# gabraham/flashpca

Measured on AMD Instinct MI355X. Metric: genotype cells/sec (N x P x iters) for k=20 PCA, higher is better.
Workload: dtype i8 (integer genotypes x 7 byte slices of the f64 operand; exact i32 accumulation, f64 recombination; agrees with the f64 kernels to ~3e-15, see fp64_mode); 1 GPU; cfg3: synthetic 500000 samples x 100000 SNPs total, SNP-sharded across GPUs, k=20 (BASELINE configs[2]/[3]); samples=500000, snps_total=100000, snps_per_gpu=100000, k=20, blockvec=16, solver_default_blockvec=16, parallelism=snp-shard x1 + all-reduce(N x b) [single]

## Files before the change

### flashpca_amd/_lib.py

```python
import ctypes as C
import os
import subprocess

HERE = os.path.dirname(os.path.abspath(__file__))
LIB_PATH = os.environ.get("FPCA_LIB") or os.path.join(HERE, "_build", "libfpca.so")
if LIB_PATH == "testhooks":
    LIB_PATH = os.path.join(HERE, "_build", "testhooks", "libfpca.so")
CLI_PATH = os.path.join(HERE, "_build", "flashpca")
HOOKS_LIB_PATH = os.path.join(HERE, "_build", "testhooks", "libfpca.so")
HOOKS_CLI_PATH = os.path.join(HERE, "_build", "testhooks", "flashpca")
CSRC = os.path.join(HERE, "csrc")

STANDARDISE = {"binom": 2, "binom2": 3}
STANDARDISE_DENSE = {"none": 0, "sd": 1, "binom": 2, "binom2": 3, "center": 4}
DIVISOR = {"none": 0, "n1": 1, "p": 2}
UNIQUE_ID_BYTES = 128
SCCA_STATUS = {0: "ok", 1: "maxiter reached", 2: "lambda1 too large", 3: "lambda2 too large"}

ALLREDUCE_FN = C.CFUNCTYPE(C.c_int, C.c_void_p, C.c_void_p, C.c_uint64, C.c_void_p)
COLLECTIVE_FN = C.CFUNCTYPE(C.c_int, C.c_void_p, C.c_void_p, C.c_void_p, C.c_uint64, C.c_void_p)


class PcaOpts(C.Structure):
    _fields_ = [
# ... 119 lines not shown
    "fpca_set_total_snps": (_I, [_P, _U64]),
    "fpca_set_rank": (_I, [_P, _I, _I]),
    "fpca_collective_stats": (_I, [_P, C.POINTER(_U64), C.POINTER(_U64)]),
    "fpca_pca_init_opts": (None, [C.POINTER(PcaOpts), C.c_size_t, C.c_size_t]),
    "fpca_pca_row_ranges": (_I, [_P, C.POINTER(PcaOpts), C.POINTER(_U64), _I]),
    "fpca_pca": (_I, [_P, C.POINTER(PcaOpts), _P, _P, _P, _P, _P, _P, C.POINTER(PcaInfo)]),
    "fpca_check": (_I, [_P, _P, C.c_int64, _P, _I, _I, _P, C.POINTER(_D), C.POINTER(_D)]),
    "fpca_ucca": (_I, [_P, _P, C.c_int64, _I, _I, _P, C.c_int64]),
    "fpca_scca_prepare": (_I, [_P, _P, C.c_int64, _I, _I, _I]),
    "fpca_scca_fit": (_I, [_P, _D, _D, _I, _I, _D, _P, C.c_int64, _P, C.c_int64, _P, C.c_int64, _P, _P, C.c_int64, _P, C.c_int64,
                           C.POINTER(_I), _P, _P, _P, C.POINTER(_I)]),
    "fpca_scca_cv": (_I, [_P, _P, C.c_int64, _I, _P, _I, _P, _I, _P, _I, _I, _I, _I, _I, _D, _P, C.c_int64, C.c_int64, _D, _I, _P, _P, _P, _P, _P, _P,
                          C.POINTER(_D), C.POINTER(_D), C.POINTER(_D), _P, _P]),
    "fpca_bench_apply": (_I, [_P, _I, _I, _I, C.POINTER(BenchResult)]),
    "fpca_profile_begin": (_I, [_P, _I]),
    "fpca_profile_sample_every": (_I, [_P, _I]),
    "fpca_profile_end": (_I, [_P, _I, C.POINTER(BenchResult), C.POINTER(_I)]),
    "fpca_bench_stats": (_I, [_P, _I, C.POINTER(_D), C.POINTER(_D)]),
    "fpca_debug_mfma_probe": (_I, [_P, _P, _P]),
    "fpca_debug_mfma_i8_probe": (_I, [_P, _P, _P]),
    "fpca_debug_mfma_peak": (_I, [_I, _I, _I, C.POINTER(_D)]),
    "fpca_debug_k4": (_I, [_P, _I, _I, _P, _P, _P, _P, _I, _P, _P]),
    "fpca_debug_k4_bench": (_I, [_P, _I, _I, _I, C.POINTER(_D), C.POINTER(_D)]),
    "fpca_debug_k4_fused": (_I, [_P, _I, _I, _P, _P, _P, _P, _P]),
    "fpca_debug_k4_fused_bench": (_I, [_P, _I, _I, _I, C.POINTER(_D)]),
    "fpca_debug_k4_inplace": (_I, [_P, _I, _I, _P, _P, _P, _I, _P, _P]),
    "fpca_debug_fp_plan": (_I, [_P, _I, C.POINTER(_I)]),
    "fpca_debug_poison_partials": (_I, [_P]),
    "fpca_debug_missing_lists": (_I, [_P, _I, _I, _P, _P, _U64, C.POINTER(_U64)]),
    "fpca_debug_gather": (_I, [_I, _I, _P, _P, _U64, _P, _U64, _P, _P, _P, _U64, _U64, _I, _D, _P, C.POINTER(_I)]),
    "fpca_debug_i8_nsc_pad": (_I, [_I, _I, C.POINTER(_I)]),
    "fpca_debug_i8_slices": (_I, [_I, _I, _I, _U64, _U64, _U64, _P, _P, _P, _P, _I, C.POINTER(SlicesOut), C.POINTER(SlicesOut), C.POINTER(_I)]),
    "fpca_debug_i8_instances": (_I, [_P, _I, C.POINTER(_I)]),
    "fpca_debug_f_sf":(_I, [_D, _U64, _I, C.POINTER(_D), C.POINTER(_D)]),
    "fpca_debug_f_sf_dev": (_I, [_P, _U64, _U64, _I, _P, _P]),
    "fpca_debug_scca_lds": (_I, [_I, C.POINTER(_I), C.POINTER(_I), C.POINTER(_I)]),
    "fpca_debug_fold_stats": (_I, [_P, _P, _I, _P, _I, _P]),
    "fpca_debug_snp_qc_rule": (_I, [_P, _P, _U64, _U64, _D, _D, _P, C.POINTER(_U64)]),
    "fpca_debug_snp_subset_bench": (_I, [_P, _P, _I, C.POINTER(_D), C.POINTER(_D)]),
    "fpca_debug_ld_prune_rule": (_I, [_P, _U64, C.c_uint32, C.c_uint32, _P, _P, _P, _P, C.POINTER(_U64)]),
    "fpca_bench_ld": (_I, [_P, C.c_uint32, _I, _P, C.POINTER(_D)]),
    "fpca_debug_king_rule": (_I, [_P, _P, _U64, _U64, _P, C.POINTER(_U64)]),
    "fpca_bench_king": (_I, [_P, _I, _P, C.POINTER(_D)]),
    "fpca_bench_king_rel": (_I, [_P, _I, _P, C.POINTER(_D)]),
    "fpca_debug_sample_qc_rule": (_I, [_P, _U64, _U64, _D, _P, C.POINTER(_U64)]),
    "fpca_debug_snp_qc_counts_rule": (_I, [_P, _P, _U64, _U64, _D, _D, _D, _P, C.POINTER(_U64)]),
    "fpca_bench_qc": (_I, [_P, _I, _P, C.POINTER(_D)]),
    "fpca_debug_scratch_live": (_I, [C.POINTER(_U64)]),
    "fpca_debug_scratch_fail_at": (_I, [_U64]),
}

ABI_VERSION = 4

_lib = None
_loaded = {}


def _load(path):
    if path not in _loaded:
        if not os.path.exists(path):
            raise RuntimeError(
                "%s not found -- build it with `make -C flashpca_amd/csrc` (or __graft_entry__.build()); this package has "
                "no CPU fallback" % path
            )
        L = C.CDLL(path)
        try:
# ... 52 lines not shown
```

### flashpca_amd/api.py

```python
import ctypes as C

import numpy as np

from . import _lib
from ._lib import DIVISOR, STANDARDISE, BenchResult, FpcaError, PcaInfo, PcaOpts, check, lib


ACCUM = {"auto": 0, 0: 0, "fp64": 64, "fp32": 32, 64: 64, 32: 32, "i8": 807}
ACCUM.update({"i8x%d" % s: 800 + s for s in range(2, 9)})
ACCUM.update({800 + s: 800 + s for s in range(2, 9)})


def _p(a):
    return a.ctypes.data_as(C.c_void_p) if a is not None else None


def count_fam_rows(path):
    with open(path, "rb") as f:
        return f.read().count(b"\n")


def _snp_mask(snps, P):
    a = np.asarray(snps)
    if a.dtype == np.bool_:
# ... 580 lines not shown
        a = dict(colmax=np.empty(64), maxbits_own=np.empty((8, 64), dtype=np.uint64), maxbits=np.empty((8, 64), dtype=np.uint64),
                 Q=np.empty((nsc, rows_pad), dtype=np.int8), colw=np.empty(nsc))
        if colsum[o]:
            a["colsum"] = np.empty((8, 640), dtype=np.int64)
        if copy[o] is not None:
            a["copy%d" % copy[o]] = np.empty((rows_pad, b), dtype=np.float32 if copy[o] == 32 else np.float64)
        if route == 1:
            a["Qrm"] = np.empty((rows_pad, S * b), dtype=np.int8)
            for w in dequant:
                a["dq%d" % w] = np.empty((rows_pad, b), dtype=np.float32 if w == 32 else np.float64)
        st = _lib.SlicesOut()
        for name, arr in a.items():
            setattr(st, name, arr.ctypes.data)
        structs.append(st)
        res.append(a)
    got = C.c_int(0)
    check(lib().fpca_debug_i8_slices(int(route), int(b), int(S), rows, rows_pad, int(rows_valid), _p(V), _p(rs[0]) if rs else None,
                                     _p(rs[1]) if len(rs) > 1 else None, _p(peers), 0 if peers is None else peers.shape[0], C.byref(structs[0]),
                                     C.byref(structs[1]) if nops > 1 else None, C.byref(got)))
    for a in res:
        a["nsc_pad"] = got.value
        if "colsum" in a:
            a["colsum_shards"] = a["colsum"]
            a["colsum"] = a["colsum_shards"].sum(axis=0)
    return res


def debug_i8_instances():
    n = C.c_int(0)
    check(lib().fpca_debug_i8_instances(None, 0, C.byref(n)))
    keys = np.zeros((n.value, 6), dtype=np.int32)
    check(lib().fpca_debug_i8_instances(_p(keys), n.value, C.byref(n)))
    return [(bool(k[0]), int(k[1]), int(k[2]), bool(k[3]), int(k[4]), bool(k[5])) for k in keys[:n.value]]


def flashpca(X, ndim=10, stand="binom2", divisor="p", maxiter=500, tol=1e-6, do_loadings=False, return_scale=True,
             device=0, verbose=False, accum="auto", keep=None, snps=None, maf=0.0, geno=1.0, ld=None, unrelated=None,
             mind=1.0, hwe=0.0, unrelated_min_shared=0, **solver_kw):
    if divisor not in DIVISOR:
        raise ValueError("divisor must be one of %s" % sorted(DIVISOR))
    qc = not (maf <= 0 and geno >= 1)
    by_mind, by_hwe = not mind >= 1, not hwe <= 0
    if (snps is not None or qc) and not isinstance(X, str):
        raise ValueError("snps / maf / geno select SNPs of a PLINK fileset; they do not apply to a numeric matrix")
    if (by_mind or by_hwe) and not isinstance(X, str):
        raise ValueError("mind / hwe filter the samples / SNPs of a PLINK fileset; they do not apply to a numeric matrix")
    if qc and keep is not None:
        raise ValueError("maf / geno cannot be combined with keep: PLINK takes these frequencies over the kept samples, the counts here "
                         "are those of all samples")
    if by_hwe and keep is not None:
        raise ValueError("hwe cannot be combined with keep: flashpca() takes the genotype counts over the samples mind= leaves; for a "
                         "hand-picked subset take the masks from qc_filter(..., keep=) and pass them as snps= and keep=")
    if ld is not None:
        ld = _ld_args(ld)
        if not isinstance(X, str):
            raise ValueError("ld prunes the SNPs of a PLINK fileset; it does not apply to a numeric matrix")
        if keep is not None:
            raise ValueError("ld cannot be combined with keep: PLINK takes r2 over the kept samples, r2 here is over all samples")
    if unrelated is not None:
        unrelated = float(unrelated)
        if not isinstance(X, str):
            raise ValueError("unrelated selects samples by the kinship of a PLINK fileset's genotypes; it does not apply to a numeric matrix")
    if isinstance(X, str):
        if stand not in STANDARDISE:
            raise ValueError("stand must be one of %s" % sorted(STANDARDISE))
        N = count_fam_rows(X + ".fam")
# ... 590 lines not shown
```

### flashpca_amd/csrc/kernels.hpp

```cpp
#pragma once
#include <hip/hip_runtime.h>

#include <cstddef>
#include <cstdint>

namespace fpca {
namespace kern {

void repitch(const uint8_t *src, uint64_t np, uint64_t nrec, uint8_t *dst, size_t pitch, hipStream_t stream);
void fix_last_byte(uint8_t *packed, size_t pitch, uint64_t np, int valid_in_last, uint64_t P_g, hipStream_t stream);
void gather_records(const uint8_t *src, size_t pitch, const uint32_t *idx, uint64_t nrec, uint8_t *dst, hipStream_t stream);
void ld_totals(const uint8_t *packed, size_t pitch, uint64_t nrec, uint32_t *tot, hipStream_t stream);
void ld_band(const uint8_t *packed, size_t pitch, const uint32_t *tot, uint32_t npad, uint64_t i0, uint64_t ni, uint64_t jend, uint32_t span,
             double *r2, uint32_t *bits, uint32_t words, double thr, bool force_general, hipStream_t stream);

void bed_stats(const uint8_t *packed, size_t pitch, uint64_t N, uint64_t P_g, int stand_method, double *lut,
               double *mean, double *sd, double *sumsq, uint32_t *nmiss , hipStream_t stream);
void lut_from_meansd(const double *mean, const double *sd, uint64_t P_g, double *lut, hipStream_t stream);

void xt_b(const uint8_t *packed, size_t pitch, const double *lut, const double *B, double *Tpart, uint64_t N_pad,
          uint64_t P_pad, int b, int nsplit, bool fp32, hipStream_t stream);
void x_t(const uint8_t *packed, size_t pitch, const double *lut, const double *T, double *Ypart, uint64_t N_pad,
         uint64_t P_pad, int b, int nsplit, bool fp32, hipStream_t stream);
void reduce_sum(const double *part, double *out, uint64_t count, int nsplit, hipStream_t stream);
// ... 41 lines not shown
                    uint32_t conc_fp = 0, uint64_t med_q32 = 0, uint32_t sig2_fp = 0);

void mfma_layout_probe(const double *A, const double *B, double *D, hipStream_t stream);

double mfma_peak_tflops(int waves_per_simd, int iters, int pattern, hipStream_t stream);

constexpr int I8_SHARDS = 8, I8_CS_STRIDE = 640;
struct SliceOp {
   const double *rowscale;
   unsigned long long *maxbits;
   int8_t *Q;
   double *colw;
   long long *colsum;
   double *copy64;
   float *copy32;
};
void i8_colmax(const double *V, uint64_t rows, int b, int nops, const SliceOp *ops, hipStream_t stream);
void i8_slice(const double *V, uint64_t rows_pad, uint64_t rows, int b, int S, int nops, const SliceOp *ops, hipStream_t stream);
void i8_maxbits_fold(const unsigned long long *bits, double *out64, hipStream_t stream);
void i8_maxbits_set(const double *all, int G, unsigned long long *bits, hipStream_t stream);
void i8_slice_rows(const double *V, uint64_t rows, int b, int S, const SliceOp &op, int8_t *Qrm, hipStream_t stream);
void i8_unpack_slices(const int8_t *Qrm, uint64_t rows_pad, int b, int S, const SliceOp &op, hipStream_t stream, uint64_t rows_valid = 0,
                      float *copy32 = nullptr, double *copy64 = nullptr);
void i8_dequant_rows(const int8_t *Qrm, uint64_t rows, int b, int S, const SliceOp &op, float *copy32, double *copy64, hipStream_t stream);
__host__ __device__ inline size_t packed_piece_offset(uint64_t r, uint64_t q, size_t pitch, bool tiled)
{
   if (!tiled) return (size_t)(r * pitch + q * 16);
   const uint64_t c = q >> 2, kh = (q >> 1) & 1, h = q & 1;
   return (size_t)((r >> 5) * 32 * pitch + c * 2048 + (h * 64 + kh * 32 + (r & 31)) * 16);
}
int gemm_i8_nsc_pad(int S, int b);
size_t gemm_i8_workspace_doubles(uint64_t rows_pad, uint64_t k_pad, int S, int b, bool two);
int gemm_i8_instances(int (*out)[6], int cap);
void gemm_i8(const uint8_t *packed, size_t pitch, const int8_t *Qg, const int8_t *Qm, const double *wg, const double *wm,
             const long long *colsum_m, const double *mean, const double *sd, double *out, double *ws, uint64_t rows_pad, uint64_t k_pad,
             uint64_t rows_valid, int mode ,
             const double *eplane , int b, int S,
             const SliceOp *next_ops, hipStream_t stream, hipEvent_t *gemm_events = nullptr, hipEvent_t before_combine = nullptr,
             bool e_only = false ,
             bool tiled = false );
void i8_rowscales(const double *mean, const double *sd, uint64_t P_g, uint64_t P_pad, double *inv_sd, double *mu_inv_sd,
                  hipStream_t stream);
void transpose_packed(const uint8_t *in, size_t pitch_in, uint64_t N_pad, uint64_t P_pad, uint8_t *out, size_t pitch_out,
                      hipStream_t stream, bool tiled = false );
void tile_packed(const uint8_t *in, size_t pitch, uint64_t rows, uint8_t *out, hipStream_t stream);
double mfma_i8_peak_tops(int waves_per_simd, int iters, uint32_t fill, hipStream_t stream);
void mfma_i8_probe(const int8_t *A, const int8_t *Bt, int *D, hipStream_t stream);

void gather_packed_rows(const uint8_t *src, size_t pitch, const uint32_t *idx, uint32_t nidx, uint32_t rows_out, uint8_t *dst, hipStream_t stream);
void patch_missing_rows(uint8_t *packed, size_t pitch, const uint32_t *idx, uint32_t nidx, hipStream_t stream);
void scatter_packed_rows(const uint8_t *src, size_t pitch, const uint32_t *idx, uint32_t nidx, uint8_t *packed, hipStream_t stream);
void gather_scaled_rows(const double *V, const double *scale, const uint32_t *idx, uint32_t nidx, uint64_t rows_out, int b, double *dst, hipStream_t stream);
void scatter_rows(const double *src, const uint32_t *idx, uint32_t nidx, int b, double *dst, hipStream_t stream);
void count_missing(const uint8_t *packed, size_t pitch, uint64_t ncols, uint64_t nrec, uint32_t *cnt, hipStream_t stream, bool tiled = false);
void fill_missing(const uint8_t *packed, size_t pitch, uint64_t ncols, uint64_t nrec, const uint32_t *ptr, uint32_t *idx, hipStream_t stream,
                  bool tiled = false);
void sparse_rows_sum(const uint32_t *ptr, const uint32_t *idx, const double *V, const double *rowscale, int b, uint64_t nrec,
                     uint64_t rows_out, double *out, hipStream_t stream, const double *init = nullptr ,
                     bool short_lists = false ,
                     double avg_len = 0 );
void sparse_rows_sum_f32(const uint32_t *ptr, const uint32_t *idx, const float *V, const double *colw, int b, uint64_t nrec, uint64_t rows_out,
                         double *out, hipStream_t stream, const double *init = nullptr, bool short_lists = false, double avg_len = 0);
int sparse_rows_sum_variant(int b, bool rowscale, bool short_lists, double avg_len);

}
}
```

### flashpca_amd/csrc/kernels_i8.hip

```cpp
#include <hip/hip_runtime.h>

#include <algorithm>
#include <cmath>
#include <cstdio>
#include <cstdlib>
#include <cstring>
#include <type_traits>
#include <utility>

#include "common.hpp"
#include "dev_scratch.hpp"
#include "kernels.hpp"
#include "launch_check.hpp"

namespace fpca {
namespace kern {

typedef int v4i __attribute__((ext_vector_type(4)));
typedef int v16i __attribute__((ext_vector_type(16)));
typedef double d2 __attribute__((ext_vector_type(2)));
typedef uint32_t u4 __attribute__((ext_vector_type(4)));
typedef uint32_t u2 __attribute__((ext_vector_type(2)));


// ... 1129 lines not shown
static int i8_bw(int b)
{
   return b == 48 ? 96 : std::max(b, 32);
}

static size_t i8_plan_doubles(const I8Plan &p, uint64_t rows_pad, int zb, int bw)
{
   return ((size_t)rows_pad + (size_t)(p.sB - 1) * p.rowsB) * zb * 2 * (size_t)bw;
}

size_t gemm_i8_workspace_doubles(uint64_t rows_pad, uint64_t k_pad, int S, int b, bool two)
{
   size_t need = 0;
   for (int mode : {(int)I8_FULL, (int)I8_SKIP_EMPTY, (int)I8_NO_MISSING}) {
      if (two && mode == I8_NO_MISSING) continue;
      const I8Shape sh = i8_shape(S, b, two, mode, rows_pad);
      const I8Plan p = i8_plan(rows_pad, k_pad, sh, i8_bw(b));
      need = std::max(need, i8_plan_doubles(p, rows_pad, sh.zb, i8_bw(b)));
   }
   return need;
}

template <class C>
static void launch_i8(const I8Plan &pl, hipStream_t stream, const uint8_t *packed, size_t pitch, const int8_t *Qg, const int8_t *Qm,
                      uint64_t k_pad, const double *wg, const double *wm, int bw, double *ws, uint64_t rows_pad, int chunks_total, int zb, uint32_t tab1)
{
   static bool attr_set = false;
   if (!attr_set) {
      (void)hipFuncSetAttribute(reinterpret_cast<const void *>(&k_gemm_i8<C>), hipFuncAttributeMaxDynamicSharedMemorySize, C::LDS_BYTES);
      attr_set = true;
   }
   hipLaunchKernelGGL(HIP_KERNEL_NAME(k_gemm_i8<C>), dim3(pl.grid), dim3(C::THREADS), C::LDS_BYTES, stream, packed, pitch, Qg, Qm, k_pad, wg, wm, bw,
                      ws, rows_pad, chunks_total, zb, pl.nA, pl.sB, pl.cpsB, pl.rowB0, pl.rowsB, tab1);
}

void gemm_i8(const uint8_t *packed, size_t pitch, const int8_t *Qg, const int8_t *Qm, const double *wg, const double *wm,
             const long long *colsum_m, const double *mean, const double *sd, double *out, double *ws, uint64_t rows_pad, uint64_t k_pad,
             uint64_t rows_valid, int mode, const double *eplane , int b,
             int S, const SliceOp *next_ops ,
             hipStream_t stream, hipEvent_t *gemm_events ,
             hipEvent_t before_combine ,
             bool e_only ,
             bool tiled )
{
   const bool two = (Qg != Qm);
   if (tiled && !two && mode != I8_NO_MISSING) throw Error(-1, "gemm_i8: the one-operand kernels of both matrices read the row-major layout only");
   if (tiled && (pitch % 64 || k_pad > 4 * pitch)) throw Error(-1, "gemm_i8: a band-tiled copy has whole 64-byte chunks per row");
   if (e_only && (mode != I8_NO_MISSING || two)) throw Error(-1, "gemm_i8: e_only goes with the one-matrix kernel");
   const I8Shape sh = i8_shape(S, b, two, mode, rows_pad);
   const int bw = i8_bw(b);
   const I8Plan pl = i8_plan(rows_pad, k_pad, sh, bw);
   const int chunks_total = (int)(k_pad / sh.kc);
   const bool nt_p = i8_nt_p(I8Key{two, mode, sh.nt, sh.half, sh.rows, tiled}, e_only);
   if (i8_verbose())
      std::fprintf(stderr, "[fpca] int8 GEMM launch: %s, mode %d, nt %d%s, %s%s; phase B from row %llu; rows %d, loads %s\n", two ? "two operands" : "one operand", mode,
                   sh.nt, sh.half ? " (half tile)" : "", tiled ? "band-tiled" : "row-major", e_only ? ", E alone" : "", (unsigned long long)pl.rowB0,
                   sh.rows, nt_p ? "p" : "plain");
   static const bool poison = FPCA_TEST_ENV("FPCA_DEBUG_I8_POISON") != nullptr;
   if (poison) {
      const size_t used = i8_plan_doubles(pl, rows_pad, sh.zb, bw);
      if (hipMemsetAsync(ws, 0xFF, used * sizeof(double), stream) != hipSuccess) throw Error(-3, "gemm_i8: poisoning the workspace failed");
   }
   if (gemm_events) (void)hipEventRecord(gemm_events[0], stream);
   if (two && mode == I8_NO_MISSING) throw Error(-1, "gemm_i8: without missing genotypes both matrices share one operand (pass Qm == Qg)");
   const bool launched = i8_find(I8Instances{}, I8Key{two, mode, sh.nt, sh.half, sh.rows, tiled, nt_p}, [&](auto c) {
      using C = decltype(c);
// ... 307 lines not shown
```

### flashpca_amd/csrc/missing_kernels.hip

```cpp
#include <hip/hip_runtime.h>

#include <algorithm>
#include <cstdlib>

#include "common.hpp"
#include "kernels.hpp"
#include "launch_check.hpp"

namespace fpca {
namespace kern {

typedef uint32_t u4 __attribute__((ext_vector_type(4)));


__global__ __launch_bounds__(256) void k_count_missing(const uint8_t *__restrict__ packed, size_t pitch, uint64_t ncols,
                                                        uint32_t *__restrict__ cnt, bool tiled)
{
   const uint64_t rec = blockIdx.x;
   auto byte_at = [&](uint64_t j) { return packed + packed_piece_offset(rec, j >> 4, pitch, tiled) + (j & 15); };
   const uint64_t nbytes = (ncols + 3) / 4, nw = nbytes / 4;
   uint32_t n = 0;
   for (uint64_t i = threadIdx.x; i < nw; i += 256) {
      const uint32_t w = *reinterpret_cast<const uint32_t *>(byte_at(4 * i));
      n += __popc(w & ~(w >> 1) & 0x55555555u);
   }
   for (uint64_t i = nw * 4 + threadIdx.x; i < nbytes; i += 256) {
      const uint32_t w = *byte_at(i);
      n += __popc(w & ~(w >> 1) & 0x55u);
   }
   if (threadIdx.x == 0 && (ncols & 3)) {
      const uint32_t w = *byte_at(nbytes - 1) >> (2 * (ncols & 3));
      n -= __popc(w & ~(w >> 1) & 0x55u);
   }
   __shared__ uint32_t red[256];
   red[threadIdx.x] = n;
   __syncthreads();
// ... 219 lines not shown
      uint32_t longest = p1 - p0;
#pragma unroll
      for (int o = 32; o >= B; o >>= 1) longest = max(longest, (uint32_t)__shfl_xor((int)longest, o));
      for (uint32_t base = 0; base < longest; base += B) {
         const uint32_t t = p0 + base + c;
         const int cnt = (int)min((uint32_t)B, p1 - p0 > base ? p1 - p0 - base : 0u);
         const uint32_t mine = t < p1 ? idx[t] : 0u;
#pragma unroll
         for (int e = 0; e < B; e += 4) {
            const uint32_t s0 = (uint32_t)__shfl((int)mine, g * B + e), s1 = (uint32_t)__shfl((int)mine, g * B + e + 1),
                           s2 = (uint32_t)__shfl((int)mine, g * B + e + 2), s3 = (uint32_t)__shfl((int)mine, g * B + e + 3);
            if (e < cnt) a0 += (double)V[(uint64_t)s0 * B + c];
            if (e + 1 < cnt) a1 += (double)V[(uint64_t)s1 * B + c];
            if (e + 2 < cnt) a2 += (double)V[(uint64_t)s2 * B + c];
            if (e + 3 < cnt) a3 += (double)V[(uint64_t)s3 * B + c];
         }
      }
      if (r < rows_out) {
         double a = (a0 + a1) + (a2 + a3);
         if (colw) a *= colw[c] * 32.0;
         out[r * B + c] = init ? init[r * B + c] + a : a;
      }
   }
}

int sparse_rows_sum_variant(int b, bool rowscale, bool short_lists, double avg_len)
{
   static const int forced = FPCA_TEST_ENV("FPCA_GATHER") ? atoi(FPCA_TEST_ENV("FPCA_GATHER")) : 0;
   const int variant = forced ? forced : (avg_len > 0 && avg_len <= 24.0 && b <= 32 && !rowscale) ? 3 : ((rowscale || short_lists) ? 2 : 1);
   if (variant == 3 && b <= 32 && !rowscale) return 3;
   return variant == 1 ? 1 : 2;
}

template <class VT>
static void sparse_rows_sum_t(const uint32_t *ptr, const uint32_t *idx, const VT *V, const double *rowscale, int b, uint64_t nrec,
                              uint64_t rows_out, double *out, hipStream_t stream, const double *init, bool short_lists, const double *colw, double avg_len)
{
   if (!rows_out) return;
   const unsigned blocks = (unsigned)std::min<uint64_t>(65536, (rows_out + 3) / 4);
   const int variant = sparse_rows_sum_variant(b, rowscale != nullptr, short_lists, avg_len);
#define FPCA_GATHER_CASE(B_)                                                                                                    \
   case B_:                                                                                                                     \
      if (variant == 3 && B_ <= 32) {                                                                                           \
         const unsigned blocks3 = (unsigned)std::min<uint64_t>(65536, (rows_out + 4 * (64 / B_) - 1) / (4 * (64 / B_)));        \
         hipLaunchKernelGGL((k_sparse_rows_sum_short<(B_ <= 32 ? B_ : 32), VT>), dim3(blocks3), dim3(256), 0, stream, ptr, idx, V, nrec, rows_out, out, init, colw); \
      } else if (variant == 1)                                                                                                  \
         hipLaunchKernelGGL((k_sparse_rows_sum<B_, VT>), dim3(blocks), dim3(256), 0, stream, ptr, idx, V, rowscale, nrec, rows_out, out, init, colw); \
      else                                                                                                                      \
         hipLaunchKernelGGL((k_sparse_rows_sum_batched<B_, VT>), dim3(blocks), dim3(256), 0, stream, ptr, idx, V, rowscale, nrec, rows_out, out, init, colw); \
      break;
   switch (b) {
      FPCA_GATHER_CASE(16)
      FPCA_GATHER_CASE(32)
      FPCA_GATHER_CASE(64)
   default: throw Error(-1, "sparse_rows_sum: block width must be 16, 32 or 64");
   }
#undef FPCA_GATHER_CASE
   launch_check();
}
void sparse_rows_sum(const uint32_t *ptr, const uint32_t *idx, const double *V, const double *rowscale, int b, uint64_t nrec,
                     uint64_t rows_out, double *out, hipStream_t stream, const double *init, bool short_lists, double avg_len)
{
   sparse_rows_sum_t<double>(ptr, idx, V, rowscale, b, nrec, rows_out, out, stream, init, short_lists, nullptr, avg_len);
}
void sparse_rows_sum_f32(const uint32_t *ptr, const uint32_t *idx, const float *V, const double *colw, int b, uint64_t nrec, uint64_t rows_out,
                         double *out, hipStream_t stream, const double *init, bool short_lists, double avg_len)
{
   sparse_rows_sum_t<float>(ptr, idx, V, nullptr, b, nrec, rows_out, out, stream, init, short_lists, colw, avg_len);
}

__global__ __launch_bounds__(256) void k_gather_packed_rows(const uint8_t *__restrict__ src, size_t pitch, const uint32_t *__restrict__ idx,
                                                             uint32_t nidx, uint8_t *__restrict__ dst)
{
   const u4 *s = blockIdx.x < nidx ? reinterpret_cast<const u4 *>(src + (size_t)idx[blockIdx.x] * pitch) : nullptr;
   u4 *d = reinterpret_cast<u4 *>(dst + (size_t)blockIdx.x * pitch);
   const u4 fill = {0xffffffffu, 0xffffffffu, 0xffffffffu, 0xffffffffu};
   for (size_t i = threadIdx.x; i < pitch / 16; i += 256) d[i] = s ? s[i] : fill;
}
__global__ __launch_bounds__(256) void k_patch_missing_rows(uint8_t *__restrict__ packed, size_t pitch, const uint32_t *__restrict__ idx)
{
   u4 *row = reinterpret_cast<u4 *>(packed + (size_t)idx[blockIdx.x] * pitch);
   for (size_t i = threadIdx.x; i < pitch / 16; i += 256) {
      u4 x = row[i];
#pragma unroll
      for (int k = 0; k < 4; k++) x[k] |= (x[k] & ~(x[k] >> 1) & 0x55555555u) << 1;
      row[i] = x;
   }
}
__global__ __launch_bounds__(256) void k_scatter_packed_rows(const uint8_t *__restrict__ src, size_t pitch, const uint32_t *__restrict__ idx,
                                                              uint8_t *__restrict__ packed)
{
   const u4 *s = reinterpret_cast<const u4 *>(src + (size_t)blockIdx.x * pitch);
   u4 *d = reinterpret_cast<u4 *>(packed + (size_t)idx[blockIdx.x] * pitch);
   for (size_t i = threadIdx.x; i < pitch / 16; i += 256) d[i] = s[i];
}
__global__ __launch_bounds__(256) void k_gather_scaled_rows(const double *__restrict__ V, const double *__restrict__ scale,
                                                             const uint32_t *__restrict__ idx, uint32_t nidx, uint64_t rows_out, int b,
                                                             double *__restrict__ dst)
{
   for (uint64_t i = (uint64_t)blockIdx.x * 256 + threadIdx.x; i < rows_out * b; i += (uint64_t)gridDim.x * 256) {
      const uint64_t r = i / b;
// ... 54 lines not shown
```

### flashpca_amd/csrc/missing_routes.hip

```cpp
#include <algorithm>
#include <cmath>

#include "ctx.hpp"

using namespace fpca;

namespace fpca {

constexpr int I8W_B = 0, I8W_G = 640, I8W_M = 1280, I8W_D = 1920, I8W_ZERO = 2560, I8W_MAXB = I8W_ZERO, I8W_MAXG = I8W_MAXB + 64 * kern::I8_SHARDS,
              I8W_MAXM = I8W_MAXG + 64 * kern::I8_SHARDS, I8W_MAXD = I8W_MAXM + 64 * kern::I8_SHARDS, I8W_CSB = I8W_MAXD + 64 * kern::I8_SHARDS,
              I8W_CSM = I8W_CSB + kern::I8_CS_STRIDE * kern::I8_SHARDS, I8W_TOTAL = I8W_CSM + kern::I8_CS_STRIDE * kern::I8_SHARDS;


constexpr double CHEAP_SPARSE_BREAK_EVEN = 0.002;
constexpr double SPARSE_BREAK_EVEN = 0.005;
static void hybrid_classify(fpca_ctx *c);
static void ensure_i8_alloc(fpca_ctx *c, int b);

static bool i8_want_tiled()
{
   const char *env = FPCA_TEST_ENV("FPCA_I8_TILED");
   return !env || atoi(env) != 0;
}

void drop_k2_copy(fpca_ctx *c, const char *why)
{
   if (c->d_packedK2) {
      (void)hipStreamSynchronize(c->stream);
      (void)hipFree(c->d_packedK2);
      c->d_packedK2 = nullptr;
   }
   c->k2_copy_failed = true;
   std::fprintf(stderr, "[fpca] no band-tiled copy of the SNP-major matrix (%.1f GiB; %s): X'B streams the row-major matrix, same results\n",
                (double)c->pitch * (double)c->P_pad / (1024.0 * 1024.0 * 1024.0), why);
}

static void ensure_k2_copy(fpca_ctx *c)
{
   if (c->d_packedK2 || c->k2_copy_failed || !c->i8_tiled) return;
   const size_t bytes = c->pitch * c->P_pad;
   size_t fr = 0, tot = 0;
   if (FPCA_TEST_ENV("FPCA_DEBUG_I8_NOK2COPY")) return drop_k2_copy(c, "FPCA_DEBUG_I8_NOK2COPY is set");
   if (hipMemGetInfo(&fr, &tot) != hipSuccess || fr < 2 * bytes) return drop_k2_copy(c, "less than twice its size is free");
   if (hipMalloc(&c->d_packedK2, bytes) != hipSuccess) {
      (void)hipGetLastError();
      c->d_packedK2 = nullptr;
      return drop_k2_copy(c, "out of device memory");
// ... 220 lines not shown
   c->hyb_class = 1;
}

int i8_mode(fpca_ctx *c, int b)
{
   const char *env = FPCA_TEST_ENV("FPCA_I8_MODE");
   const bool sparse_ok = c->missing_known && !c->sparse_failed && c->n_missing < (1ull << 31) && (b == 16 || b == 32 || b == 64);
   const bool lists_ok = c->missing_known && !c->sparse_failed && (b == 16 || b == 32 || b == 64);
   if (env && atoi(env) == I8M_HYBRID) {
      hybrid_classify(c);
      return (lists_ok && c->hyb_class == 1 && !c->hyb_failed) ? I8M_HYBRID : I8M_FULL;
   }
   if (env) return (atoi(env) == I8M_SPARSE && !sparse_ok) ? I8M_FULL : atoi(env);
   if (!c->missing_known) return I8M_FULL;
   if (c->n_missing == 0) return I8M_NONE;
   const double rate = (double)c->n_missing / ((double)c->N * (double)std::max<uint64_t>(c->P_g, 1));
   if (lists_ok && !c->hyb_failed) {
      hybrid_classify(c);
      if (c->hyb_class == 1) return I8M_HYBRID;
   }
   if (sparse_ok && rate <= SPARSE_BREAK_EVEN) {
      if (c->i8_Sc > 0 && c->i8_Sc < c->i8_S && c->i8_Sc <= 4 && rate > CHEAP_SPARSE_BREAK_EVEN && !c->hyb_view) return I8M_FULL;
      return I8M_SPARSE;
   }
   return rate < 3e-4 ? I8M_SKIP : I8M_FULL;
}

bool sparse_on_side_stream(const fpca_ctx *c, int b)
{
   static const double thr = FPCA_TEST_ENV("FPCA_SPARSE_SIDE_BYTES") ? atof(FPCA_TEST_ENV("FPCA_SPARSE_SIDE_BYTES")) : 2e9;
   return (double)(c->hyb_view ? c->hyb_sparse_nnz : c->n_missing) * b * 8.0 > thr;
}

void ensure_sparse(fpca_ctx *c, int b)
{
   hipStream_t s = c->stream;
   const size_t need = (size_t)std::max(c->N_pad, c->P_pad) * b;
   if (FPCA_TEST_ENV("FPCA_DEBUG_SPARSE_NOMEM")) throw Error(FPCA_ENOMEM, "FPCA_DEBUG_SPARSE_NOMEM is set");
   if (need > c->eplane_cap) {
      if (c->d_eplane) HIP_CHECK(hipFree(c->d_eplane));
      c->d_eplane = nullptr;
      c->eplane_cap = 0;
      HIP_ALLOC(hipMalloc(&c->d_eplane, 2 * need * sizeof(double)));
      c->eplane_cap = need;
   }
   if (c->sparse_ready) return;
   if (!c->aux_stream) {
      int lo = 0, hi = 0;
      (void)hipDeviceGetStreamPriorityRange(&lo, &hi);
      HIP_CHECK(hipStreamCreateWithPriority(&c->aux_stream, hipStreamNonBlocking, lo));
      HIP_CHECK(hipEventCreateWithFlags(&c->ev_aux_go, hipEventDisableTiming));
      HIP_CHECK(hipEventCreateWithFlags(&c->ev_aux_done, hipEventDisableTiming));
   }
   const uint64_t nnz = c->hyb_view ? c->hyb_sparse_nnz : c->n_missing;
   std::vector<uint32_t> ptr(c->P_g + 1, 0);
   {
      size_t d = 0;
      for (uint64_t j = 0; j < c->P_g; j++) {
         const bool dense = c->hyb_view && d < c->h_hyb_idx.size() && c->h_hyb_idx[d] == j;
         if (dense) d++;
         ptr[j + 1] = ptr[j] + (dense ? 0u : c->h_nmiss[j]);
      }
   }
   HIP_ALLOC(hipMalloc(&c->d_snp_ptr, (c->P_g + 1) * sizeof(uint32_t)));
   HIP_ALLOC(hipMalloc(&c->d_snp_idx, std::max<uint64_t>(nnz, 1) * sizeof(uint32_t)));
   HIP_CHECK(hipMemcpyAsync(c->d_snp_ptr, ptr.data(), (c->P_g + 1) * sizeof(uint32_t), hipMemcpyHostToDevice, s));
// ... 124 lines not shown
}

void xt_i8(fpca_ctx *c, const double *dB, int b, hipStream_t s, bool chain, hipEvent_t *gev, const PreSliced *pre)
{
   kern::SliceOp ob = i8_op_b(c), ot[2];
   if (pre) {
      ob.maxbits = pre->maxbits;
      ob.colw = pre->colw;
   }
   i8_ops_t(c, ot);
   int mode = i8_mode(c, b);
   const double *eplane = nullptr;
   hipEvent_t wait = nullptr;
   if (mode == I8M_SPARSE || mode == I8M_HYBRID)
      mode = sparse_or_dense(c, b, mode);
   else
      plain_view(c);
   const bool hyb = mode == I8M_HYBRID;
   const bool g32 = (mode == I8M_SPARSE || hyb) && c->gather_f32();
   if (g32) ob.copy32 = static_cast<float *>(c->gather_src());
   if (pre) {
      const bool gathers = mode == I8M_SPARSE || hyb;
      kern::i8_unpack_slices(pre->Qrm, c->N_pad, b, c->cur_S(), ob, s, c->N, (gathers && g32) ? ob.copy32 : nullptr, (gathers && !g32) ? pre->dq64 : nullptr);
      if (gathers && !g32) dB = pre->dq64;
   } else {
      kern::i8_colmax(dB, c->N, b, 1, &ob, s);
      kern::i8_slice(dB, c->N_pad, c->N, b, c->cur_S(), 1, &ob, s);
   }
   if (hyb)
      kern::gemm_i8(c->d_packedE, c->pitch, c->d_Qb, c->d_Qb, ob.colw, ob.colw, nullptr, nullptr, nullptr, c->d_hyb_plane, c->d_i8ws, c->hyb_pad, c->N_pad,
                    c->hyb_n, I8M_NONE, nullptr, b, c->cur_S(), nullptr, s, nullptr, nullptr, true);
   if (mode == I8M_SPARSE || hyb) {
      hipStream_t gs = s;
      if (sparse_on_side_stream(c, b)) {
         HIP_CHECK(hipEventRecord(c->ev_aux_go, s));
         HIP_CHECK(hipStreamWaitEvent(c->aux_stream, c->ev_aux_go, 0));
         gs = c->aux_stream;
      }
      if (g32)
         kern::sparse_rows_sum_f32(c->d_snp_ptr, c->d_snp_idx, ob.copy32, ob.colw, b, c->P_g, c->P_pad, c->d_eplane, gs);
      else
         kern::sparse_rows_sum(c->d_snp_ptr, c->d_snp_idx, dB, nullptr, b, c->P_g, c->P_pad, c->d_eplane, gs);
      if (hyb) kern::scatter_rows(c->d_hyb_plane, c->d_hyb_idx, c->hyb_n, b, c->d_eplane, gs);
      if (gs != s) {
         HIP_CHECK(hipEventRecord(c->ev_aux_done, c->aux_stream));
         wait = c->ev_aux_done;
      }
      eplane = c->d_eplane;
      mode = I8M_NONE;
   }
   const bool k2t = c->d_packedK2 && mode == I8M_NONE;
   kern::gemm_i8(k2t ? c->d_packedK2 : c->d_packed, c->pitch, c->d_Qb, c->d_Qb, ob.colw, ob.colw, ob.colsum, c->d_mean, c->d_sd, c->d_T, c->d_i8ws, c->P_pad,
                 c->N_pad, c->P_g, mode, eplane, b, c->cur_S(), chain ? ot : nullptr, s, gev, wait, false, k2t);
}

void x_i8(fpca_ctx *c, int b, double *dY, hipStream_t s, bool have_max, bool do_slice, uint64_t r0, uint64_t r1, hipEvent_t *gev)
{
   kern::SliceOp ot[2];
   i8_ops_t(c, ot);
   int mode = i8_mode(c, b);
   if (mode == I8M_SPARSE || mode == I8M_HYBRID)
      mode = sparse_or_dense(c, b, mode);
   else
      plain_view(c);
   const bool hyb = mode == I8M_HYBRID;
   if (hyb) mode = I8M_SPARSE;
   if (do_slice) {
      if (!have_max) kern::i8_colmax(c->d_T, c->P_g, b, 2, ot, s);
      const bool g32 = c->gather_f32();
      if (mode == I8M_SPARSE) {
         if (g32)
            ot[1].copy32 = static_cast<float *>(c->gather_src());
         else
            ot[1].copy64 = static_cast<double *>(c->gather_src());
      }
      kern::i8_slice(c->d_T, c->P_pad, c->P_g, b, c->cur_S(), 2, ot, s);
      if (hyb) {
         kern::SliceOp od{nullptr, reinterpret_cast<unsigned long long *>(c->d_i8w + I8W_MAXD), c->d_Qd, c->d_i8w + I8W_D, nullptr};
         kern::gather_scaled_rows(c->d_T, c->d_mu_inv_sd, c->d_hyb_idx, c->hyb_n, c->hyb_pad, b, c->d_hyb_T, s);
         kern::i8_colmax(c->d_hyb_T, c->hyb_n, b, 1, &od, s);
         kern::i8_slice(c->d_hyb_T, c->hyb_pad, c->hyb_n, b, c->cur_S(), 1, &od, s);
         kern::gemm_i8(c->d_packedET, c->pitchET, c->d_Qd, c->d_Qd, od.colw, od.colw, nullptr, nullptr, nullptr, c->d_hyb_plane, c->d_i8ws, c->N_pad,
                       c->hyb_pad, c->N, I8M_NONE, nullptr, b, c->cur_S(), nullptr, s, nullptr, nullptr, true);
      }
      const double *init = hyb ? c->d_hyb_plane : nullptr;
      if (mode == I8M_SPARSE) {
         hipStream_t gs = s;
         const double per_sample = (double)(c->hyb_view ? c->hyb_sparse_nnz : c->n_missing) / (double)std::max<uint64_t>(c->N, 1);
         if (sparse_on_side_stream(c, b)) {
            HIP_CHECK(hipEventRecord(c->ev_aux_go, s));
            HIP_CHECK(hipStreamWaitEvent(c->aux_stream, c->ev_aux_go, 0));
            gs = c->aux_stream;
         }
         if (g32)
            kern::sparse_rows_sum_f32(c->d_smp_ptr, c->d_smp_idx, ot[1].copy32, ot[1].colw, b, c->N, c->N_pad, c->d_eplane, gs, init, true, per_sample);
         else
            kern::sparse_rows_sum(c->d_smp_ptr, c->d_smp_idx, ot[1].copy64, nullptr, b, c->N, c->N_pad, c->d_eplane, gs, init, true, per_sample);
         if (gs != s) HIP_CHECK(hipEventRecord(c->ev_aux_done, c->aux_stream));
      }
   }
   if (r1 == 0) r1 = c->N_pad;
   if (r1 <= r0) return;
   const double *eplane = nullptr;
   hipEvent_t wait = nullptr;
   if (mode == I8M_SPARSE) {
      eplane = c->d_eplane + r0 * b;
      if (sparse_on_side_stream(c, b)) wait = c->ev_aux_done;
      mode = I8M_NONE;
   }
   if (c->i8_tiled && r0 % 32) throw Error(-1, "x_i8: a row range of the band-tiled copy starts at a multiple of 32 rows");
   kern::gemm_i8(c->d_packedT + r0 * c->pitchT, c->pitchT, c->d_Qg, mode == I8M_NONE ? c->d_Qg : c->d_Qm, ot[0].colw, ot[1].colw,
                 ot[1].colsum, nullptr, nullptr, dY + r0 * b, c->d_i8ws, r1 - r0, c->P_pad, c->N > r0 ? std::min(c->N - r0, r1 - r0) : 0, mode,
                 eplane, b, c->cur_S(), nullptr, s, gev, wait, false, c->i8_tiled);
}

}
```

### include/fpca_debug.h

```cpp
#ifndef FPCA_DEBUG_H
#define FPCA_DEBUG_H

#include "fpca.h"

#ifdef __cplusplus
extern "C" {
#endif

typedef struct fpca_bench_result {
   double ms_total;
   double ms_xt;
   double ms_x;
   double ms_allreduce;
   double flops_per_step;
   double packed_bytes_per_step;
   double ms_gemm_xt;
   double ms_gemm_x;
} fpca_bench_result;
int fpca_bench_apply(fpca_ctx *ctx, int b, int steps, int warmup, fpca_bench_result *res);
int fpca_profile_begin(fpca_ctx *ctx, int max_steps);
int fpca_profile_sample_every(fpca_ctx *ctx, int stride);
int fpca_profile_end(fpca_ctx *ctx, int b, fpca_bench_result *res, int *nsteps);
int fpca_bench_stats(fpca_ctx *ctx, int reps, double *ms_per_launch, double *bytes_per_launch);

// ... 4 lines not shown
                  double *Out, double *G_out);
int fpca_debug_k4_fused(fpca_ctx *ctx, int b, int nq, const double *V, const double *W, const double *C_in, double *Out, double *Cg);
int fpca_debug_k4_fused_bench(fpca_ctx *ctx, int b, int nq, int reps, double *ms_fused);
int fpca_debug_k4_inplace(fpca_ctx *ctx, int b, int nq, const double *V, const double *W, const double *C_in, int mode, double *Out,
                          double *G_out);
int fpca_debug_k4_bench(fpca_ctx *ctx, int b, int nq, int reps, double *ms_gram, double *ms_gemm);

int fpca_debug_fp_plan(fpca_ctx *ctx, int b, int out[6]);
int fpca_debug_poison_partials(fpca_ctx *ctx);

int fpca_debug_missing_lists(fpca_ctx *ctx, int b, int by_sample, uint32_t *ptr_out, uint32_t *idx_out, uint64_t idx_cap, uint64_t *nnz);
int fpca_debug_gather(int b, int use_f32, const uint32_t *ptr, const uint32_t *idx, uint64_t nnz, const void *V, uint64_t v_rows,
                      const double *rowscale, const double *colw, const double *init, uint64_t nrec, uint64_t rows_out, int short_lists,
                      double avg_len, double *out, int *variant);

typedef struct fpca_debug_slices_out {
   double *colmax;
   uint64_t *maxbits_own;
   uint64_t *maxbits;
   int8_t *Q;
   int8_t *Qrm;
   double *colw;
   int64_t *colsum;
   float *copy32;
   double *copy64;
   float *dq32;
   double *dq64;
} fpca_debug_slices_out;
int fpca_debug_i8_nsc_pad(int S, int b, int *nsc_pad);
int fpca_debug_i8_slices(int route, int b, int S, uint64_t rows, uint64_t rows_pad, uint64_t rows_valid, const double *V, const double *rowscale0,
                         const double *rowscale1, const double *peers, int n_peers, fpca_debug_slices_out *out0, fpca_debug_slices_out *out1,
                         int *nsc_pad);
int fpca_debug_i8_instances(int32_t *keys, int cap, int *count);

int fpca_debug_f_sf(double r2, uint64_t n, int k, double *F, double *P);
int fpca_debug_f_sf_dev(const double *r2, uint64_t count, uint64_t n, int k, double *F, double *P);
int fpca_debug_scca_lds(int device, int *max_k, int *need_at_max_k, int *per_workgroup);
int fpca_debug_fold_stats(fpca_ctx *ctx, const uint8_t *fold, int nfolds, uint32_t *counts, int which_fold, double *mean_sd);
int fpca_debug_snp_qc_rule(const double *mean, const uint32_t *n_missing, uint64_t N, uint64_t P, double min_maf, double max_missing,
                           uint8_t *keep, uint64_t *n_kept);
int fpca_debug_snp_subset_bench(fpca_ctx *src, const uint8_t *keep, int reps, double *ms_per_launch, double *bytes_per_launch);
int fpca_debug_ld_prune_rule(const uint32_t *bits, uint64_t P, uint32_t window, uint32_t step, const uint64_t *totals, const double *maf,
                             const uint32_t *chrom, uint8_t *keep, uint64_t *n_kept);
int fpca_bench_ld(fpca_ctx *ctx, uint32_t span, int reps, double *ms, double *macs);
int fpca_debug_king_rule(const uint32_t *i, const uint32_t *j, uint64_t n_pairs, uint64_t N, uint8_t *keep, uint64_t *n_kept);
int fpca_bench_king(fpca_ctx *ctx, int reps, double *ms, double *macs);
int fpca_bench_king_rel(fpca_ctx *ctx, int reps, double *ms, double *macs);
int fpca_debug_sample_qc_rule(const uint32_t *counts, uint64_t n_snps, uint64_t N, double max_missing, uint8_t *samples, uint64_t *n_kept);
int fpca_debug_snp_qc_counts_rule(const uint32_t *counts, const double *p_hwe, uint64_t n, uint64_t P, double min_maf, double max_missing,
                                  double min_hwe_p, uint8_t *keep, uint64_t *n_kept);
int fpca_bench_qc(fpca_ctx *ctx, int reps, double *ms, double *hwe_steps);

int fpca_debug_scratch_live(uint64_t out[3]);
int fpca_debug_scratch_fail_at(uint64_t n);

#ifdef __cplusplus
}
#endif
#endif
```

Baseline: 79420 billion cells/s.

## Size side-stream gather grid to CU slots left by the concurrent i8 GEMM

When the sparse missing-genotype gather runs on the auxiliary stream beside the i8 GEMM, its grid is now capped at the number of blocks that fit in the wave slots and VGPRs the GEMM workgroups leave free on each CU. The cap uses the GEMM instance's waves, registers and LDS and the gather kernel's register count. The aim is to keep the gather from crowding GEMM workgroups off CUs. It also raises the cheap-sparse break-even threshold, so more missingness cases take the sparse route. The cost is a possibly slower gather when few blocks fit. The synthetic benchmark likely has no or few missing genotypes, so this path may not run.

```diff
diff --git a/flashpca_amd/_lib.py b/flashpca_amd/_lib.py
--- a/flashpca_amd/_lib.py
+++ b/flashpca_amd/_lib.py
@@ -175,6 +175,7 @@
     "fpca_debug_i8_nsc_pad": (_I, [_I, _I, C.POINTER(_I)]),
     "fpca_debug_i8_slices": (_I, [_I, _I, _I, _U64, _U64, _U64, _P, _P, _P, _P, _I, C.POINTER(SlicesOut), C.POINTER(SlicesOut), C.POINTER(_I)]),
     "fpca_debug_i8_instances": (_I, [_P, _I, C.POINTER(_I)]),
+    "fpca_debug_gather_blocks": (_I, [_I, _I, _I, _I, _I, _U64, C.POINTER(C.c_uint32), C.POINTER(C.c_uint32), C.POINTER(C.c_uint32)]),
     "fpca_debug_f_sf":(_I, [_D, _U64, _I, C.POINTER(_D), C.POINTER(_D)]),
     "fpca_debug_f_sf_dev": (_I, [_P, _U64, _U64, _I, _P, _P]),
     "fpca_debug_scca_lds": (_I, [_I, C.POINTER(_I), C.POINTER(_I), C.POINTER(_I)]),
diff --git a/flashpca_amd/api.py b/flashpca_amd/api.py
--- a/flashpca_amd/api.py
+++ b/flashpca_amd/api.py
@@ -636,6 +636,13 @@
     keys = np.zeros((n.value, 6), dtype=np.int32)
     check(lib().fpca_debug_i8_instances(_p(keys), n.value, C.byref(n)))
     return [(bool(k[0]), int(k[1]), int(k[2]), bool(k[3]), int(k[4]), bool(k[5])) for k in keys[:n.value]]
+
+
+def debug_gather_blocks(gemm_waves, gemm_vgprs, gemm_lds, gather_vgprs, ncu, rows_out=1 << 30):
+    lim, side, inline = C.c_uint32(0), C.c_uint32(0), C.c_uint32(0)
+    check(lib().fpca_debug_gather_blocks(int(gemm_waves), int(gemm_vgprs), int(gemm_lds), int(gather_vgprs), int(ncu), int(rows_out),
+                                         C.byref(lim), C.byref(side), C.byref(inline)))
+    return lim.value, side.value, inline.value
 
 
 def flashpca(X, ndim=10, stand="binom2", divisor="p", maxiter=500, tol=1e-6, do_loadings=False, return_scale=True,
diff --git a/flashpca_amd/csrc/kernels.hpp b/flashpca_amd/csrc/kernels.hpp
--- a/flashpca_amd/csrc/kernels.hpp
+++ b/flashpca_amd/csrc/kernels.hpp
@@ -97,6 +97,10 @@
 int gemm_i8_nsc_pad(int S, int b);
 size_t gemm_i8_workspace_doubles(uint64_t rows_pad, uint64_t k_pad, int S, int b, bool two);
 int gemm_i8_instances(int (*out)[6], int cap);
+struct CuFootprint {
+   int waves, vgprs, lds_bytes;
+};
+CuFootprint gemm_i8_footprint(uint64_t rows_pad, int S, int b, bool two, int mode, bool e_only, bool tiled);
 void gemm_i8(const uint8_t *packed, size_t pitch, const int8_t *Qg, const int8_t *Qm, const double *wg, const double *wm,
              const long long *colsum_m, const double *mean, const double *sd, double *out, double *ws, uint64_t rows_pad, uint64_t k_pad,
              uint64_t rows_valid, int mode ,
@@ -123,10 +127,15 @@
 void sparse_rows_sum(const uint32_t *ptr, const uint32_t *idx, const double *V, const double *rowscale, int b, uint64_t nrec,
                      uint64_t rows_out, double *out, hipStream_t stream, const double *init = nullptr ,
                      bool short_lists = false ,
-                     double avg_len = 0 );
+                     double avg_len = 0 ,
+                     unsigned block_limit = 0 );
 void sparse_rows_sum_f32(const uint32_t *ptr, const uint32_t *idx, const float *V, const double *colw, int b, uint64_t nrec, uint64_t rows_out,
-                         double *out, hipStream_t stream, const double *init = nullptr, bool short_lists = false, double avg_len = 0);
+                         double *out, hipStream_t stream, const double *init = nullptr, bool short_lists = false, double avg_len = 0,
+                         unsigned block_limit = 0);
 int sparse_rows_sum_variant(int b, bool rowscale, bool short_lists, double avg_len);
+unsigned gather_blocks_beside(const CuFootprint &gemm, int gather_vgprs, int ncu);
+unsigned sparse_rows_sum_grid(uint64_t rows_out, unsigned block_limit);
+unsigned sparse_rows_sum_blocks_beside(const CuFootprint &gemm, int b, bool f32, bool rowscale, bool short_lists, double avg_len);
 
 }
 }
diff --git a/flashpca_amd/csrc/kernels_i8.hip b/flashpca_amd/csrc/kernels_i8.hip
--- a/flashpca_amd/csrc/kernels_i8.hip
+++ b/flashpca_amd/csrc/kernels_i8.hip
@@ -1185,6 +1185,25 @@
    }
    hipLaunchKernelGGL(HIP_KERNEL_NAME(k_gemm_i8<C>), dim3(pl.grid), dim3(C::THREADS), C::LDS_BYTES, stream, packed, pitch, Qg, Qm, k_pad, wg, wm, bw,
                       ws, rows_pad, chunks_total, zb, pl.nA, pl.sB, pl.cpsB, pl.rowB0, pl.rowsB, tab1);
+}
+
+CuFootprint gemm_i8_footprint(uint64_t rows_pad, int S, int b, bool two, int mode, bool e_only, bool tiled)
+{
+   const I8Shape sh = i8_shape(S, b, two, mode, rows_pad);
+   const bool nt_p = i8_nt_p(I8Key{two, mode, sh.nt, sh.half, sh.rows, tiled}, e_only);
+   CuFootprint f{0, 0, 0};
+   i8_find(I8Instances{}, I8Key{two, mode, sh.nt, sh.half, sh.rows, tiled, nt_p}, [&](auto c) {
+      using C = decltype(c);
+      static int regs = 0;
+      if (!regs) {
+         hipFuncAttributes attr;
+         regs = hipFuncGetAttributes(&attr, reinterpret_cast<const void *>(&k_gemm_i8<C>)) == hipSuccess && attr.numRegs > 0 ? attr.numRegs : 256;
+      }
+      f = CuFootprint{C::WAVES, regs, C::LDS_BYTES};
+      return true;
+   });
+   if (!f.waves) throw Error(-1, "gemm_i8: no kernel instance for this shape");
+   return f;
 }
 
 void gemm_i8(const uint8_t *packed, size_t pitch, const int8_t *Qg, const int8_t *Qm, const double *wg, const double *wm,
diff --git a/flashpca_amd/csrc/missing_kernels.hip b/flashpca_amd/csrc/missing_kernels.hip
--- a/flashpca_amd/csrc/missing_kernels.hip
+++ b/flashpca_amd/csrc/missing_kernels.hip
@@ -1,7 +1,10 @@
 #include <hip/hip_runtime.h>
 
 #include <algorithm>
+#include <cstdio>
 #include <cstdlib>
+#include <map>
+#include <mutex>
 
 #include "common.hpp"
 #include "kernels.hpp"
@@ -287,13 +290,71 @@
    return variant == 1 ? 1 : 2;
 }
 
+unsigned gather_blocks_beside(const CuFootprint &gemm, int gather_vgprs, int ncu)
+{
+   constexpr int SIMDS = 4, WAVE_SLOTS = 8, VGPRS = 512, LDS = 160 * 1024;
+   const auto alloc = [](int r) { return (std::max(r, 1) + 7) / 8 * 8; };
+   const int wps = std::max((gemm.waves + SIMDS - 1) / SIMDS, 1), regs = alloc(gemm.vgprs) * wps;
+   const int wgs = std::max(std::min({WAVE_SLOTS / wps, VGPRS / regs, gemm.lds_bytes > 0 ? LDS / gemm.lds_bytes : WAVE_SLOTS}), 1);
+   const int slots = WAVE_SLOTS - wgs * wps, left = VGPRS - wgs * regs;
+   const int per_cu = std::min(slots, left / alloc(gather_vgprs));
+   return (unsigned)std::max(per_cu, 1) * (unsigned)std::max(ncu, 1);
+}
+
+unsigned sparse_rows_sum_grid(uint64_t rows_out, unsigned block_limit)
+{
+   const unsigned blocks = (unsigned)std::min<uint64_t>(65536, (rows_out + 3) / 4);
+   return block_limit ? std::min(blocks, block_limit) : blocks;
+}
+
+template <class VT>
+static const void *sparse_rows_sum_kernel(int variant, int b)
+{
+#define FPCA_GATHER_FN(B_) (variant == 1 ? reinterpret_cast<const void *>(&k_sparse_rows_sum<B_, VT>) : reinterpret_cast<const void *>(&k_sparse_rows_sum_batched<B_, VT>))
+   return b == 16 ? FPCA_GATHER_FN(16) : b == 32 ? FPCA_GATHER_FN(32) : b == 64 ? FPCA_GATHER_FN(64) : nullptr;
+#undef FPCA_GATHER_FN
+}
+
+unsigned sparse_rows_sum_blocks_beside(const CuFootprint &gemm, int b, bool f32, bool rowscale, bool short_lists, double avg_len)
+{
+   const int variant = sparse_rows_sum_variant(b, rowscale, short_lists, avg_len);
+   if (variant == 3) return 0;
+   const void *fn = f32 ? sparse_rows_sum_kernel<float>(variant, b) : sparse_rows_sum_kernel<double>(variant, b);
+   if (!fn) throw Error(-1, "sparse_rows_sum: block width must be 16, 32 or 64");
+   static std::mutex mtx;
+   static std::map<const void *, int> regs_of;
+   static int ncu = 0;
+   std::lock_guard<std::mutex> lock(mtx);
+   auto it = regs_of.find(fn);
+   if (it == regs_of.end()) {
+      hipFuncAttributes attr;
+      if (hipFuncGetAttributes(&attr, fn) != hipSuccess || attr.numRegs <= 0) throw Error(-3, "sparse_rows_sum: the gather kernel's registers could not be read");
+      it = regs_of.emplace(fn, attr.numRegs).first;
+   }
+   if (!ncu) {
+      int dev = 0;
+      if (hipGetDevice(&dev) != hipSuccess || hipDeviceGetAttribute(&ncu, hipDeviceAttributeMultiprocessorCount, dev) != hipSuccess || ncu <= 0) {
+         ncu = 0;
+         throw Error(-3, "sparse_rows_sum: the device's CU count could not be read");
+      }
+   }
+   return gather_blocks_beside(gemm, it->second, ncu);
+}
+
 template <class VT>
 static void sparse_rows_sum_t(const uint32_t *ptr, const uint32_t *idx, const VT *V, const double *rowscale, int b, uint64_t nrec,
-                              uint64_t rows_out, double *out, hipStream_t stream, const double *init, bool short_lists, const double *colw, double avg_len)
+                              uint64_t rows_out, double *out, hipStream_t stream, const double *init, bool short_lists, const double *colw, double avg_len,
+                              unsigned block_limit)
 {
    if (!rows_out) return;
-   const unsigned blocks = (unsigned)std::min<uint64_t>(65536, (rows_out + 3) / 4);
+   if (const char *env_b = FPCA_TEST_ENV("FPCA_GATHER_BLOCKS")) {
+      if (atoi(env_b) < 0) throw Error(-1, "FPCA_GATHER_BLOCKS is a number of blocks (0: no limit)");
+      block_limit = (unsigned)atoi(env_b);
+   }
+   const unsigned blocks = sparse_rows_sum_grid(rows_out, block_limit);
    const int variant = sparse_rows_sum_variant(b, rowscale != nullptr, short_lists, avg_len);
+   if (FPCA_TEST_ENV("FPCA_GATHER_VERBOSE"))
+      std::fprintf(stderr, "[fpca] gather launch: kernel %d, %llu rows, %u blocks, limit %u\n", variant, (unsigned long long)rows_out, blocks, block_limit);
 #define FPCA_GATHER_CASE(B_)                                                                                                    \
    case B_:                                                                                                                     \
       if (variant == 3 && B_ <= 32) {                                                                                           \
@@ -314,14 +375,14 @@
    launch_check();
 }
 void sparse_rows_sum(const uint32_t *ptr, const uint32_t *idx, const double *V, const double *rowscale, int b, uint64_t nrec,
-                     uint64_t rows_out, double *out, hipStream_t stream, const double *init, bool short_lists, double avg_len)
-{
-   sparse_rows_sum_t<double>(ptr, idx, V, rowscale, b, nrec, rows_out, out, stream, init, short_lists, nullptr, avg_len);
+                     uint64_t rows_out, double *out, hipStream_t stream, const double *init, bool short_lists, double avg_len, unsigned block_limit)
+{
+   sparse_rows_sum_t<double>(ptr, idx, V, rowscale, b, nrec, rows_out, out, stream, init, short_lists, nullptr, avg_len, block_limit);
 }
 void sparse_rows_sum_f32(const uint32_t *ptr, const uint32_t *idx, const float *V, const double *colw, int b, uint64_t nrec, uint64_t rows_out,
-                         double *out, hipStream_t stream, const double *init, bool short_lists, double avg_len)
-{
-   sparse_rows_sum_t<float>(ptr, idx, V, nullptr, b, nrec, rows_out, out, stream, init, short_lists, colw, avg_len);
+                         double *out, hipStream_t stream, const double *init, bool short_lists, double avg_len, unsigned block_limit)
+{
+   sparse_rows_sum_t<float>(ptr, idx, V, nullptr, b, nrec, rows_out, out, stream, init, short_lists, colw, avg_len, block_limit);
 }
 
 __global__ __launch_bounds__(256) void k_gather_packed_rows(const uint8_t *__restrict__ src, size_t pitch, const uint32_t *__restrict__ idx,
diff --git a/flashpca_amd/csrc/missing_routes.hip b/flashpca_amd/csrc/missing_routes.hip
--- a/flashpca_amd/csrc/missing_routes.hip
+++ b/flashpca_amd/csrc/missing_routes.hip
@@ -12,7 +12,7 @@
               I8W_CSM = I8W_CSB + kern::I8_CS_STRIDE * kern::I8_SHARDS, I8W_TOTAL = I8W_CSM + kern::I8_CS_STRIDE * kern::I8_SHARDS;
 
 
-constexpr double CHEAP_SPARSE_BREAK_EVEN = 0.002;
+constexpr double CHEAP_SPARSE_BREAK_EVEN = 0.0035;
 constexpr double SPARSE_BREAK_EVEN = 0.005;
 static void hybrid_classify(fpca_ctx *c);
 static void ensure_i8_alloc(fpca_ctx *c, int b);
@@ -299,6 +299,14 @@
    return (double)(c->hyb_view ? c->hyb_sparse_nnz : c->n_missing) * b * 8.0 > thr;
 }
 
+constexpr double RESIDENT_GATHER_MAX_RATE = 0.003;
+static unsigned side_gather_blocks(const fpca_ctx *c, const kern::CuFootprint &gemm, int b, bool f32, bool short_lists, double avg_len)
+{
+   const double listed = (double)(c->hyb_view ? c->hyb_sparse_nnz : c->n_missing);
+   if (listed > RESIDENT_GATHER_MAX_RATE * (double)c->N * (double)std::max<uint64_t>(c->P_g, 1)) return 0;
+   return kern::sparse_rows_sum_blocks_beside(gemm, b, f32, false, short_lists, avg_len);
+}
+
 void ensure_sparse(fpca_ctx *c, int b)
 {
    hipStream_t s = c->stream;
@@ -489,15 +497,17 @@
                     c->hyb_n, I8M_NONE, nullptr, b, c->cur_S(), nullptr, s, nullptr, nullptr, true);
    if (mode == I8M_SPARSE || hyb) {
       hipStream_t gs = s;
+      unsigned limit = 0;
       if (sparse_on_side_stream(c, b)) {
          HIP_CHECK(hipEventRecord(c->ev_aux_go, s));
          HIP_CHECK(hipStreamWaitEvent(c->aux_stream, c->ev_aux_go, 0));
          gs = c->aux_stream;
+         limit = side_gather_blocks(c, kern::gemm_i8_footprint(c->P_pad, c->cur_S(), b, false, I8M_NONE, false, c->d_packedK2 != nullptr), b, g32, false, 0.0);
       }
       if (g32)
-         kern::sparse_rows_sum_f32(c->d_snp_ptr, c->d_snp_idx, ob.copy32, ob.colw, b, c->P_g, c->P_pad, c->d_eplane, gs);
+         kern::sparse_rows_sum_f32(c->d_snp_ptr, c->d_snp_idx, ob.copy32, ob.colw, b, c->P_g, c->P_pad, c->d_eplane, gs, nullptr, false, 0, limit);
       else
-         kern::sparse_rows_sum(c->d_snp_ptr, c->d_snp_idx, dB, nullptr, b, c->P_g, c->P_pad, c->d_eplane, gs);
+         kern::sparse_rows_sum(c->d_snp_ptr, c->d_snp_idx, dB, nullptr, b, c->P_g, c->P_pad, c->d_eplane, gs, nullptr, false, 0, limit);
       if (hyb) kern::scatter_rows(c->d_hyb_plane, c->d_hyb_idx, c->hyb_n, b, c->d_eplane, gs);
       if (gs != s) {
          HIP_CHECK(hipEventRecord(c->ev_aux_done, c->aux_stream));
@@ -543,16 +553,19 @@
       const double *init = hyb ? c->d_hyb_plane : nullptr;
       if (mode == I8M_SPARSE) {
          hipStream_t gs = s;
+         unsigned limit = 0;
          const double per_sample = (double)(c->hyb_view ? c->hyb_sparse_nnz : c->n_missing) / (double)std::max<uint64_t>(c->N, 1);
          if (sparse_on_side_stream(c, b)) {
             HIP_CHECK(hipEventRecord(c->ev_aux_go, s));
             HIP_CHECK(hipStreamWaitEvent(c->aux_stream, c->ev_aux_go, 0));
             gs = c->aux_stream;
+            const uint64_t rend = r1 ? r1 : c->N_pad, rows = rend > r0 ? rend - r0 : c->N_pad;
+            limit = side_gather_blocks(c, kern::gemm_i8_footprint(rows, c->cur_S(), b, false, I8M_NONE, false, c->i8_tiled), b, g32, true, per_sample);
          }
          if (g32)
-            kern::sparse_rows_sum_f32(c->d_smp_ptr, c->d_smp_idx, ot[1].copy32, ot[1].colw, b, c->N, c->N_pad, c->d_eplane, gs, init, true, per_sample);
+            kern::sparse_rows_sum_f32(c->d_smp_ptr, c->d_smp_idx, ot[1].copy32, ot[1].colw, b, c->N, c->N_pad, c->d_eplane, gs, init, true, per_sample, limit);
          else
-            kern::sparse_rows_sum(c->d_smp_ptr, c->d_smp_idx, ot[1].copy64, nullptr, b, c->N, c->N_pad, c->d_eplane, gs, init, true, per_sample);
+            kern::sparse_rows_sum(c->d_smp_ptr, c->d_smp_idx, ot[1].copy64, nullptr, b, c->N, c->N_pad, c->d_eplane, gs, init, true, per_sample, limit);
          if (gs != s) HIP_CHECK(hipEventRecord(c->ev_aux_done, c->aux_stream));
       }
    }
diff --git a/include/fpca_debug.h b/include/fpca_debug.h
--- a/include/fpca_debug.h
+++ b/include/fpca_debug.h
@@ -60,6 +60,8 @@
                          const double *rowscale1, const double *peers, int n_peers, fpca_debug_slices_out *out0, fpca_debug_slices_out *out1,
                          int *nsc_pad);
 int fpca_debug_i8_instances(int32_t *keys, int cap, int *count);
+int fpca_debug_gather_blocks(int gemm_waves, int gemm_vgprs, int gemm_lds, int gather_vgprs, int ncu, uint64_t rows_out, uint32_t *limit,
+                             uint32_t *grid_side, uint32_t *grid_inline);
 
 int fpca_debug_f_sf(double r2, uint64_t n, int k, double *F, double *P);
 int fpca_debug_f_sf_dev(const double *r2, uint64_t count, uint64_t n, int k, double *F, double *P);
```

Result: faster. 80840 billion cells/s (median of 6 runs) (+1.8%).
